# shz9/viprs

Hardware: AMD Instinct MI355X
Metric: SNP-updates/sec/E-step (1M SNPs, ~1700 LD blocks) (higher is better)
Workload: dtype f32

## Files before the change

viprs_amd/csrc/estep_panel.h:

```cpp
#pragma once
#include <type_traits>

#include "device_math.h"
#include "kernels_common.h"
#include "panel_loads.h"
#include "panel_models.h"

#ifndef PANEL_MIN_WAVES
#define PANEL_MIN_WAVES 2
#endif

namespace viprs {

#ifdef VIPRS_SWEEP_TRACE
__device__ unsigned long long g_sweep_trace[1 << 15][4];
__device__ unsigned int g_sweep_trace_n;
#endif

#ifdef VIPRS_PANEL_PROFILE
#define PPROF(slot, cond) do { if (TEAM && item == 0 && member < 2 && lane == 0 && p < 64 && (cond)) s_pprof[p][slot] = (unsigned)wall_clock64(); } while (0)
#else
#define PPROF(slot, cond) do { } while (0)
#endif

template <typename U> __host__ __device__ constexpr int panel_cols() { return sizeof(U) == 4 ? 4 : 8; }
template <typename U> __host__ __device__ constexpr int panel_team_cols() {
#ifdef PANEL_TEAM_CPL_F32
    return sizeof(U) == 4 ? PANEL_TEAM_CPL_F32 : 4;
#else
    return sizeof(U) == 4 ? 2 : 4;
#endif
}

constexpr int kFormSym = 1, kFormMirror = 2;

template <typename U, typename MODEL, int FORM, int NW, bool TEAM, int CPL>
__device__ __forceinline__ void panel_role(const EStepArgs<float>& A0, const int qcap, float* __restrict__ smem, const int wg) {
    constexpr bool MIR = FORM == kFormMirror;
    constexpr bool SUMS = FORM != kFormSym;
    const PanelLds lds(qcap, MODEL::kLaneParallel && !is_wide_mixture<MODEL>::value, MIR);
    float* lq = smem + lds.q();
    float* la = smem + lds.a();
    float* lT = smem + lds.diag_tiles();
    float* lTo = smem + lds.offdiag_tile();
    float* lmx = smem + lds.mix();
    float* led = smem + lds.ed();
    float* ls = smem + lds.s();
#ifdef PANEL_TEAM_STRIP_DEPTH
    constexpr int kDepth = TEAM ? PANEL_TEAM_STRIP_DEPTH : kStripRowsInFlight;
#else
    constexpr int kDepth = TEAM ? (kPanel / RawRow<U, CPL>::kWords < kPanel ? kPanel / RawRow<U, CPL>::kWords : kPanel) : kStripRowsInFlight;
#endif
    __shared__ int s_blk;
    __shared__ int s_tdone;
    __shared__ int s_ddone;

    const int tid = threadIdx.x;
    const int wave = __builtin_amdgcn_readfirstlane(tid >> 6);
    const int lane = tid & 63;
    const U* __restrict__ ldd = static_cast<const U*>(A0.ld_dense);
    ExpTab tab;
    tab.init();
    unsigned long long my_skipped = 0;
    const float dq = A0.dq;
    const int n_models = max(1, A0.n_active);

    constexpr int kSW = kPanel * CPL;
    const int TS = TEAM ? A0.team_size : 1;
    const int team = TEAM ? wg / TS : 0;
    const int member = TEAM ? wg % TS : 0;
    int team_iter = 0;

    for (;;) {
        int item;
        if (TEAM) {
            item = team + team_iter * A0.n_teams;
            ++team_iter;
        } else {
            if (tid == 0) {
                int it = atomicAdd(A0.counter, 1);
                if (A0.bottom_mod > 0 && it < A0.n_blocks * n_models) {
                    const bool bottom = (wg % A0.bottom_mod) == A0.bottom_mod - 1;
                    it = bottom ? A0.n_blocks * n_models - 1 - atomicAdd(A0.counter + 2, 1) : atomicAdd(A0.counter + 1, 1);
                }
                s_blk = it;
            }
            __syncthreads();
            item = s_blk;
            __syncthreads();
        }
        if (item >= A0.n_blocks * n_models) break;
        const int blk = item / n_models, model_slot = item - blk * n_models;
        if constexpr (IsGridColumn<MODEL>::value) {
            if (A0.group_cols) {
                const int on = A0.group_cols[(int64_t)A0.blk_group[blk] * A0.width + A0.active[model_slot]];
                if (__builtin_amdgcn_readfirstlane(on) == 0) continue;
            }
        }
        const EStepArgs<float> A = select_model(A0, model_slot);

        const BlockDesc bd = A.blocks[blk];
        const int64_t s0 = bd.start;
        const int b = bd.size;
#ifdef VIPRS_SWEEP_TRACE
        const unsigned long long trace_t0 = wall_clock64();
#endif
        unsigned long long* __restrict__ gran =
            TEAM ? A.granules + ((int64_t)model_slot * A.granule_rows + bd.gr_off) * kPanel : nullptr;
        const int stride = bd.stride;
        const U* __restrict__ base = ldd + bd.ld_off;
        const int np = (b + kPanel - 1) / kPanel;
        const int bpad = np * kPanel;
        const int nstrips_all = (bpad + kSW - 1) / kSW;
        const int n_own = TEAM ? (nstrips_all - member + TS - 1) / TS : nstrips_all;
        auto own = [&](int c) { return !TEAM || ((c / kSW) % TS) == member; };
        auto loc = [&](int c) { return TEAM ? ((c / kSW) / TS) * kSW + (c % kSW) : c; };
        auto glob = [&](int li) { return TEAM ? ((li / kSW) * TS + member) * kSW + (li % kSW) : li; };

        for (int li = tid; li < (TEAM ? n_own * kSW : bpad) + kStrip; li += NW * 64) {
            const int c = glob(li);
            const bool in = (!TEAM || li < n_own * kSW) && c < b;
            lq[li] = in ? A.q[s0 + c] : 0.0f;
            if (SUMS) ls[li] = 0.0f;
        }
        if (tid == 0) { s_tdone = 0; s_ddone = 0; }
        for (int i = tid; i < kPanel * kPanel / 4; i += NW * 64) {
            const int row = i >> 4, tcol = (i & 15) * 4;
            *reinterpret_cast<float4*>(lT + row * kPanel + tcol) = load4<U>(base + (int64_t)min(row, b - 1) * stride + tcol);
        }
        __syncthreads();

        float a_prev = 0.0f;

        typename MODEL::In nxt_in{};
        if (wave == 0) {
            const bool live0 = lane < b;
            nxt_in = MODEL::load(A, s0 + (live0 ? lane : 0), live0);
        }

#ifdef VIPRS_PANEL_PROFILE
        __shared__ unsigned s_pprof[64][8];
#endif
        if (wave == 0) {
#ifdef PANEL_CHAIN_PRIO
        __builtin_amdgcn_s_setprio(PANEL_CHAIN_PRIO);
#endif
        for (int p = 0; p < np + 1; ++p) {
            PPROF(0, true);
            {
                if (p < np) {
                    const int r0 = p * kPanel;
                    const int nrows = min(kPanel, b - r0);
                    const int64_t j = s0 + r0 + lane;
                    const bool live = lane < nrows;
                    const typename MODEL::In in = nxt_in;
                    {
                        const int rn = r0 + kPanel + lane;
                        const bool ln = rn < b;
                        nxt_in = MODEL::load(A, s0 + (ln ? rn : 0), ln);
                    }

                    float qc;
                    float q_own = 0.0f;
                    if (own(r0)) qc = lq[loc(r0 + lane)];
                    else qc = (r0 + lane < b) ? A.q[s0 + r0 + lane] : 0.0f;
                    if (TEAM && p >= 2 && (((p * kPanel) / kSW) % TS) != member) {
                        unsigned long long g = 0;
#ifdef PANEL_TIMING_NO_HANDOFF_WAIT
                        if (false)
#endif
                        for (unsigned spins = 0;; ++spins) {
                            g = __hip_atomic_load(gran + (int64_t)p * kPanel + lane, __ATOMIC_RELAXED,
                                                  __HIP_MEMORY_SCOPE_AGENT);
                            if (__all((unsigned)(g >> 32) == A.tag_base + (unsigned)(p + 1))) break;
                            if (spins > (1u << 22)) {
                                if (lane == 0) atomicExch(A.error, 1);
                                break;
                            }
                            if ((spins & 1023u) == 1023u &&
                                __hip_atomic_load(A.error, __ATOMIC_RELAXED, __HIP_MEMORY_SCOPE_AGENT) != 0) break;
                            __builtin_amdgcn_s_sleep(8);
                        }
                        qc = __uint_as_float((unsigned)g);
                    }
                    PPROF(1, true);
                    if (p > 0) {
                        {
                            float trow[kPanel];
#pragma unroll
                            for (int k = 0; k < kPanel; ++k) trow[k] = lTo[k * kPanel + lane];
                            if constexpr (sizeof(U) < 4 || MODEL::kLaneParallel) {
                                const float4* __restrict__ av4 = reinterpret_cast<const float4*>(la + ((p - 1) & 1) * kPanel);
                                float4 av[kPanel / 4];
#pragma unroll
                                for (int i = 0; i < kPanel / 4; ++i) av[i] = av4[i];
#pragma unroll
                                for (int k = 0; k < kPanel; ++k) {
                                    const float4 t = av[k >> 2];
                                    const float ak = (k & 3) == 0 ? t.x : (k & 3) == 1 ? t.y : (k & 3) == 2 ? t.z : t.w;
                                    qc = __builtin_fmaf(trow[k], ak, qc);
                                }
                            } else {
#pragma unroll
                                for (int k = 0; k < kPanel; ++k) qc = __builtin_fmaf(trow[k], rl(a_prev, k), qc);
                            }
                        }
                    }

                    {
                        if (lane == 0) *reinterpret_cast<volatile int*>(&s_tdone) = p + 1;
                    }
                    PPROF(2, true);
                    if constexpr (is_wide_mixture<MODEL>::value) {
                        constexpr int KMAX = MODEL::kMax;
                        const int K = in.K;
                        const int kc = min(lane, K - 1);
                        const bool comp = lane < K;
                        float dvec = 0.0f, avec = 0.0f;
                        const int64_t jlast = s0 + b - 1;
                        auto cptr = [&](const float* __restrict__ arr, int jj) {
                            return arr + min(s0 + r0 + jj, jlast) * K + kc;
                        };
                        static_assert(kChainPrefetch == 16 && kPanel == 64, "window indexing");
                        float rmm[kChainPrefetch], rsv[kChainPrefetch], rul[kChainPrefetch];
                        float rvec = in.beta - qc;
                        const float* __restrict__ DtW = lT + (p & 1) * kPanel * kPanel + lane;
#pragma unroll
                        for (int k = 0; k < kChainPrefetch; ++k) {
                            rmm[k] = *cptr(A.mu_mult, k);
                            rsv[k] = *cptr(A.shvt, k);
                            rul[k] = *cptr(A.u_logs, k);
                        }
#pragma unroll 1
                        for (int g = 0; g < kPanel / kChainPrefetch; ++g) {
#pragma unroll
                        for (int k = 0; k < kChainPrefetch; ++k) {
                            const int jj = kChainPrefetch * g + k;
                            const float drow_jj = DtW[jj * kPanel];
                            const float cmm = rmm[k], csv = rsv[k], cul = rul[k];
                            {
                                rmm[k] = *cptr(A.mu_mult, jj + kChainPrefetch);
                                rsv[k] = *cptr(A.shvt, jj + kChainPrefetch);
                                rul[k] = *cptr(A.u_logs, jj + kChainPrefetch);
                            }
                            const float lnp = rl(in.lnp, jj), eta_old = rl(in.eta_old, jj);
                            const float r = rl(rvec, jj);
                            const float mu = cmm * r;
                            const float t = csv * mu;
                            float u = __builtin_fmaf(t, t, cul);
                            u = (lane == K) ? lnp : u;
                            float mx = dpp_max_shr<1>(u);
                            mx = dpp_max_shr<2>(mx);
                            mx = dpp_max_shr<4>(mx);
                            mx = dpp_max_shr<8>(mx);
                            const float m_lo = rl(mx, 15), m_hi = rl(mx, K);
                            mx = (K >= 16) ? fmaxf(m_lo, m_hi) : m_hi;
                            float e = expf_glibc_nonpos<kLookupPerLane>(u - mx, tab);
                            e = (lane <= K) ? e : 0.0f;
                            static_assert((KMAX + 1) % 8 == 0, "chunks of 8 terms");
                            float ssum = 0.0f;
#pragma unroll
                            for (int c = 0; c < (KMAX + 1) / 8; ++c) {
                                int et[8];
#pragma unroll
                                for (int i = 0; i < 8; ++i) et[i] = __builtin_amdgcn_readlane(__float_as_int(e), 8 * c + i);
                                pin_sgprs(et);
#pragma unroll
                                for (int i = 0; i < 8; ++i) ssum = (c == 0 && i == 0) ? __int_as_float(et[0]) : ssum + __int_as_float(et[i]);
                            }
                            const float gam = comp ? e / ssum : 0.0f;
                            float d = -eta_old;
#pragma unroll
                            for (int c = 0; c < (KMAX + 1) / 8; ++c) {
                                int gt[8];
                                float mb[8];
#pragma unroll
                                for (int i = 0; i < 8; ++i) {
                                    gt[i] = __builtin_amdgcn_readlane(__float_as_int(gam), 8 * c + i);
                                    mb[i] = rl(mu, 8 * c + i);
                                }
                                pin_sgprs(gt);
#pragma unroll
                                for (int i = 0; i < 8; ++i) d = __builtin_fmaf(__int_as_float(gt[i]), mb[i], d);
                            }
                            const bool livej = jj < nrows;
                            const float a = livej ? dq * d : 0.0f;
                            if (comp && livej && member == 0) {
                                const int64_t o = (s0 + r0 + jj) * K + lane;
                                A.var_mu[o] = mu;
                                A.var_gamma[o] = gam;
                            }
                            int l = lane;
                            asm volatile("" : "+v"(l));
                            const bool me = (l == jj);
                            dvec = me ? d : dvec;
                            avec = me ? a : avec;
                            if (MIR) q_own = me ? qc : q_own;
                            qc = __builtin_fmaf(drow_jj, a, qc);
                            rvec = in.beta - qc;
                            if (!MIR) qc = (me && livej) ? qc - d : qc;
                        }
                        }
                        if (member == 0 && live) {
                            A.eta_diff[j] = dvec;
                            if (TEAM) stage_store(A.eta_out + j, in.eta_old + dvec); else A.eta[j] = in.eta_old + dvec;
                        }
                        a_prev = avec;
                        if (SUMS) led[(p & 1) * kPanel + lane] = live ? dvec : 0.0f;
                    } else if constexpr (MODEL::kLaneParallel) {
                        const int K = in.K;
                        float* __restrict__ Lmm = lmx;
                        float* __restrict__ Lsv = lmx + kPanel * kPanelMaxK;
                        float* __restrict__ Lul = lmx + 2 * kPanel * kPanelMaxK;
                        float* __restrict__ Lmu = lmx + 3 * kPanel * kPanelMaxK;
                        float* __restrict__ Lga = lmx + 4 * kPanel * kPanelMaxK;
#pragma unroll
                        for (int k = 0; k < kPanelMaxK; ++k) {
                            if (k < K) {
                                Lmm[lane * K + k] = in.mm[k];
                                Lsv[lane * K + k] = in.sv[k];
                                Lul[lane * K + k] = in.ulog[k];
                            }
                        }
                        __builtin_amdgcn_wave_barrier();
                        const int kc = min(lane, K - 1);
                        float cmm = Lmm[kc], csv = Lsv[kc], cul = Lul[kc];
                        float dvec = 0.0f, avec = 0.0f;
                        auto run_panel = [&](auto rounds_c, auto k4_c) {
                        constexpr int ROUNDS = decltype(rounds_c)::value;
                        constexpr bool K4 = decltype(k4_c)::value;
                        float rvec = in.beta - qc;
                        static_assert(kChainPrefetch == 16 && kPanel == 64, "group indexing");
                        const float* __restrict__ Dt = lT + (p & 1) * kPanel * kPanel + lane;
#pragma unroll 1
                        for (int g = 0; g < kPanel / kChainPrefetch; ++g) {
#pragma unroll
                        for (int k = 0; k < kChainPrefetch; ++k) {
                            const int jj = kChainPrefetch * g + k;
                            const float drow_jj = Dt[jj * kPanel];
                            const int jn = (jj + 1 < kPanel) ? jj + 1 : jj;
                            const float nmm = Lmm[jn * K + kc], nsv = Lsv[jn * K + kc], nul = Lul[jn * K + kc];
                            const float lnp = rl(in.lnp, jj), eta_old = rl(in.eta_old, jj);
                            const float r = rl(rvec, jj);
                            const float mu = cmm * r;
                            const float t = csv * mu;
                            float u = __builtin_fmaf(t, t, cul);
                            u = (lane == K) ? lnp : u;
                            float mub[ROUNDS];
#pragma unroll
                            for (int i = 0; i < ROUNDS; ++i) mub[i] = rl(mu, i);
                            float mx;
                            if constexpr (K4) {
                                int ut[5];
#pragma unroll
                                for (int i = 0; i < 5; ++i) ut[i] = __builtin_amdgcn_readlane(__float_as_int(u), i);
                                pin_sgprs(ut);
                                mx = __int_as_float(ut[0]);
#pragma unroll
                                for (int i = 1; i <= 4; ++i) mx = fmaxf(mx, __int_as_float(ut[i]));
                            } else {
                                mx = dpp_max_shr<1>(u);
                                mx = dpp_max_shr<2>(mx);
                                mx = dpp_max_shr<4>(mx);
                                mx = dpp_max_shr<8>(mx);
                                mx = rl(mx, K);
                            }
                            const float e = softmax_exp<MODEL::kExact, kLookupPerLane>(u - mx, tab);
                            const float e_t = (K4 || lane <= K) ? e : 0.0f;
                            int et[ROUNDS + 1];
#pragma unroll
                            for (int i = 0; i <= ROUNDS; ++i) et[i] = __builtin_amdgcn_readlane(__float_as_int(e_t), i);
                            pin_sgprs(et);
                            float ssum = __int_as_float(et[0]);
#pragma unroll
                            for (int i = 1; i <= ROUNDS; ++i) ssum += __int_as_float(et[i]);
                            const float gam = softmax_div<MODEL::kExact>(e, ssum);
                            const float gam_t = (K4 || lane < K) ? gam : 0.0f;
                            int gt[ROUNDS];
#pragma unroll
                            for (int i = 0; i < ROUNDS; ++i) gt[i] = __builtin_amdgcn_readlane(__float_as_int(gam_t), i);
                            pin_sgprs(gt);
                            float d = -eta_old;
#pragma unroll
                            for (int i = 0; i < ROUNDS; ++i) d = __builtin_fmaf(__int_as_float(gt[i]), mub[i], d);
                            const bool livej = jj < nrows;
                            const float a = livej ? dq * d : 0.0f;
                            if (lane < K) {
                                Lmu[jj * K + lane] = mu;
                                Lga[jj * K + lane] = gam;
                            }
                            int l = lane;
                            asm volatile("" : "+v"(l));
                            const bool me = (l == jj);
                            dvec = me ? d : dvec;
                            avec = me ? a : avec;
                            if (MIR) q_own = me ? qc : q_own;
                            qc = __builtin_fmaf(drow_jj, a, qc);
                            rvec = in.beta - qc;
                            if (!MIR) qc = (me && livej) ? qc - d : qc;
                            cmm = nmm; csv = nsv; cul = nul;
                        }
                        }
                        };
                        if (K == 4) run_panel(std::integral_constant<int, 4>{}, std::true_type{});
                        else if (K < 4) run_panel(std::integral_constant<int, 4>{}, std::false_type{});
                        else run_panel(std::integral_constant<int, kPanelMaxK>{}, std::false_type{});
                        __builtin_amdgcn_wave_barrier();
                        if (member == 0) {
                            const int64_t o = (s0 + r0) * K;
                            for (int i = lane; i < nrows * K; i += 64) {
                                A.var_mu[o + i] = Lmu[i];
                                A.var_gamma[o + i] = Lga[i];
                            }
                            if (live) {
                                A.eta_diff[j] = dvec;
                                if (TEAM) stage_store(A.eta_out + j, in.eta_old + dvec); else A.eta[j] = in.eta_old + dvec;
                            }
                        }
                        a_prev = avec;
                        if (SUMS) led[(p & 1) * kPanel + lane] = live ? dvec : 0.0f;
                    } else {
                        float qcap_v = 0.0f;
                        const float* __restrict__ Dt = lT + (p & 1) * kPanel * kPanel + lane;
                        unsigned long long lane_bit = 1ull;
                        float qf = qc;
    #pragma unroll
                        for (int jj = 0; jj < kPanel; ++jj) {
                            const float dr = Dt[jj * kPanel];
                            const float d = MODEL::template delta<kLookupLane>(in, qf, tab, jj);
                            const float dz = (MODEL::kHasSkip && fabsf(d) < Eps<float>::value) ? 0.0f : d;
                            const float az = dq * dz;
                            const float sa = rl(az, jj);
                            const float sdz = rl(dz, jj);
                            qcap_v = sel_mask(qcap_v, qc, lane_bit);
                            qf = __builtin_fmaf(dr, sa, qc);
                            qc = !MIR ? sel_mask(qf, qf - sdz, lane_bit) : qf;
                            asm volatile("s_lshl_b64 %0, %0, 1" : "+s"(lane_bit) : : "scc");
                        }
                        q_own = qcap_v;

                        PPROF(3, true);
                        bool skipped_lane;
                        float d_lane = 0.0f;
                        a_prev = MODEL::template finish<TEAM>(A, j, in, qcap_v, tab, live, member == 0, skipped_lane, &d_lane);
                        my_skipped += __popcll(__ballot(skipped_lane));
                        if (SUMS) led[(p & 1) * kPanel + lane] = d_lane;
                    }
                    la[(p & 1) * kPanel + lane] = a_prev;
                    if (own(r0)) lq[loc(r0 + lane)] = MIR ? q_own : qc;
                    PPROF(4, true);
                }
            }
            __syncthreads();
        }
        } else {
        for (int p = 0; p < np + 1; ++p) {
            {
                const int uw = wave - 1;
                auto stage_tiles = [&]() {
                if (p + 1 < np) {
                    float* __restrict__ T = lT + ((p + 1) & 1) * kPanel * kPanel;
                    const int trow = lane >> 4, tcol = (lane & 15) * 4;
                    const int row_base = (p + 1) * kPanel;
                    constexpr int kGroups = (kPanel / 4 + NW - 2) / (NW - 1);
                    float4 v[kGroups];
#pragma unroll
                    for (int g = 0; g < kGroups; ++g) {
                        const int row = 4 * min(uw + g * (NW - 1), kPanel / 4 - 1) + trow;
                        v[g] = load4<U>(base + (int64_t)min(row_base + row, b - 1) * stride + (p + 1) * kPanel + tcol);
                    }
                    float4 w[kGroups];
                    {
#pragma unroll
                        for (int g = 0; g < kGroups; ++g) {
                            const int row = 4 * min(uw + g * (NW - 1), kPanel / 4 - 1) + trow;
                            w[g] = load4<U>(base + (int64_t)min(p * kPanel + row, b - 1) * stride + (p + 1) * kPanel + tcol);
                        }
                    }
                    if (MIR && p > 0) {
                        while (*reinterpret_cast<volatile int*>(&s_ddone) < p) __builtin_amdgcn_s_sleep(1);
                    }
#pragma unroll
                    for (int g = 0; g < kGroups; ++g) {
                        const int i = uw + g * (NW - 1);
                        if (i < kPanel / 4) *reinterpret_cast<float4*>(T + (4 * i + trow) * kPanel + tcol) = v[g];
                    }
                    {
                        while (*reinterpret_cast<volatile int*>(&s_tdone) < p + 1) __builtin_amdgcn_s_sleep(1);
#pragma unroll
                        for (int g = 0; g < kGroups; ++g) {
                            const int i = uw + g * (NW - 1);
                            if (i < kPanel / 4) *reinterpret_cast<float4*>(lTo + (4 * i + trow) * kPanel + tcol) = w[g];
                        }
                    }
                }
                };
                const int pp = p - 1;
                const int rr0 = pp * kPanel;
                const int last_row = min(kPanel, b - rr0) - 1;
                const float avec = p > 0 ? la[(pp & 1) * kPanel + lane] : 0.0f;
                const int nstrips = (bpad + kSW - 1) / kSW;
                const bool any_a = __ballot(avec != 0.0f) != 0;
                const float edvec = (MIR && p > 0) ? led[(pp & 1) * kPanel + lane] : 0.0f;
                const bool any_ed = MIR && __ballot(edvec != 0.0f) != 0;
                const int s_pri = ((p + 1) * kPanel) / kSW;
                const int n_mine = (nstrips - member + TS - 1) / TS;
                auto do_strip = [&](int k) {
                    int st = member + k * TS, kl = k;
                    if (TEAM) {
                        const int k_pri = (s_pri % TS == member) ? (s_pri - member) / TS : 0;
                        kl = (k + k_pri) % n_mine;
                        st = member + kl * TS;
                    }
                    const int c = st * kSW + CPL * lane;
                    float* __restrict__ lq_c = lq + (TEAM ? kl * kSW + CPL * lane : c);
                    const int cp = c >> 6;
#if defined(PANEL_TIMING_NO_SECOND_PASS) && PANEL_TIMING_NO_SECOND_PASS + 0 >= 2
                    const bool active = (c < b) && cp > p;
#else
                    const bool active = (c < b) && cp != pp && cp != p;
#endif
                    auto hand_off = [&]() {
                        if (TEAM && st == s_pri && p + 1 < np && p + 1 >= 2) {
                            __builtin_amdgcn_wave_barrier();
                            const float v = lq[loc((p + 1) * kPanel + lane)];
                            const unsigned long long g =
                                ((unsigned long long)(A.tag_base + (unsigned)(p + 2)) << 32) | (unsigned long long)__float_as_uint(v);
                            __hip_atomic_store(gran + (int64_t)(p + 1) * kPanel + lane, g, __ATOMIC_RELAXED,
                                               __HIP_MEMORY_SCOPE_AGENT);
                        }
                    };
                    if constexpr (MIR) {
                        const bool left = cp < pp;
                        float* __restrict__ tgt = left ? ls + (TEAM ? kl * kSW + CPL * lane : c) : lq_c;
                        const bool any_l = __ballot(active && left) != 0, any_r = __ballot(active && !left) != 0;
                        if (any_l && any_r) {
                            const float fvec = left ? 1.0f : dq;
                            if (any_ed && active) {
                                if (last_row == kPanel - 1)
                                    strip_update<U, CPL, true, kDepth, true>(base + (int64_t)rr0 * stride + c, stride, last_row, edvec, tgt, fvec);
                                else
                                    strip_update<U, CPL, false, kDepth, true>(base + (int64_t)rr0 * stride + c, stride, last_row, edvec, tgt, fvec);
                            }
                        } else {
                            float mvec = any_l ? edvec : avec;
                            asm volatile("" : "+v"(mvec));
                            if ((any_l ? any_ed : any_a) && active) {
                                if (last_row == kPanel - 1)
                                    strip_update<U, CPL, true, kDepth>(base + (int64_t)rr0 * stride + c, stride, last_row, mvec, tgt);
                                else
                                    strip_update<U, CPL, false, kDepth>(base + (int64_t)rr0 * stride + c, stride, last_row, mvec, tgt);
                            }
                        }
                        if (k == uw) PPROF(6, wave == 1);
                        hand_off();
                    } else {
                        if (any_a && active) {
                            if (last_row == kPanel - 1)
                                strip_update<U, CPL, true, kDepth>(base + (int64_t)rr0 * stride + c, stride, last_row, avec, lq_c);
                            else
                                strip_update<U, CPL, false, kDepth>(base + (int64_t)rr0 * stride + c, stride, last_row, avec, lq_c);
                        }
                        if (k == uw) PPROF(6, wave == 1);
                        hand_off();
                    }
                };
                if (MIR && p > 0 && uw == NW - 2) {
#ifdef PANEL_TIMING_NO_SECOND_PASS
                    if (false) {
#else
                    if (any_ed && own(rr0)) {
#endif
                        float* __restrict__ sp = ls + loc(rr0 + lane);
                        *sp = diag_lower_update(lT + (pp & 1) * kPanel * kPanel, edvec, *sp, lane);
                    }
                    if (lane == 0) *reinterpret_cast<volatile int*>(&s_ddone) = p;
                }
                stage_tiles();
                PPROF(5, wave == 1);
                if (p > 0) {
                    for (int k = uw; k < n_mine; k += NW - 1) do_strip(k);
                }
            }
            PPROF(7, wave == 1);
            __syncthreads();
        }
        }
#ifdef VIPRS_PANEL_PROFILE
        if (TEAM && item == 0 && member < 2 && tid == 0) {
            for (int p = 0; p < np && p < 64; p += (p < 4 || p > np - 4) ? 1 : 8) {
                const unsigned t = s_pprof[p][0];
                printf("m%d phase %2d @%7u: granule %4d T-apply %4d loop %5d replay %5d end %5d | upd: staged %5d pri %5d all %5d (x10ns)\n",
                       member, p, t - s_pprof[0][0], (int)(s_pprof[p][1] - t), (int)(s_pprof[p][2] - t), (int)(s_pprof[p][3] - t),
                       (int)(s_pprof[p][4] - t), (int)(s_pprof[p][4] - t), (int)(s_pprof[p][5] - t), (int)(s_pprof[p][6] - t),
                       (int)(s_pprof[p][7] - t));
            }
        }
#endif
        {
            for (int li = tid; li < (TEAM ? n_own * kSW : b); li += NW * 64) {
                const int i = glob(li);
                if (i < b) {
                    const float v = SUMS ? lq[li] + A.dq * ls[li] : lq[li];
                    if (TEAM) stage_store(A.q_out + s0 + i, v); else A.q[s0 + i] = v;
                }
            }
        }
        if (TEAM) {
            asm volatile("s_waitcnt vmcnt(0)" ::: "memory");
            __syncthreads();
            if (tid == 0) s_blk = (atomicAdd(A.arrive + item, 1) == TS - 1) ? 1 : 0;
            __syncthreads();
            const bool last = s_blk != 0;
            if (last) {
                for (int i = tid; i < b; i += NW * 64) {
                    A.eta[s0 + i] = __hip_atomic_load(A.eta_out + s0 + i, __ATOMIC_RELAXED, __HIP_MEMORY_SCOPE_AGENT);
                    A.q[s0 + i] = __hip_atomic_load(A.q_out + s0 + i, __ATOMIC_RELAXED, __HIP_MEMORY_SCOPE_AGENT);
                }
                if (tid == 0) atomicExch(A.arrive + item, 0);
            }
        }
        __syncthreads();
#ifdef VIPRS_SWEEP_TRACE
        if (tid == 0) {
            const unsigned k = atomicAdd(&g_sweep_trace_n, 1u);
            if (k < (1u << 15)) {
                g_sweep_trace[k][0] = ((unsigned long long)blockIdx.x << 32) | (unsigned)(TEAM ? 1 : 0);
                g_sweep_trace[k][1] = (unsigned long long)b;
                g_sweep_trace[k][2] = trace_t0;
                g_sweep_trace[k][3] = wall_clock64();
            }
        }
#endif
    }
    if (lane == 0 && my_skipped && member == 0) atomicAdd(A0.skipped, my_skipped);
}

struct SweepArgs {
    EStepArgs<float> cls[3];
    int32_t qcap[3];
    int32_t n_wg[2];
    int32_t narrow0;
    int32_t* done;
    unsigned long long* skipped_last;
};

template <typename U, typename MODEL, int FORM, int NW, int CPL>
__global__ __launch_bounds__(NW * 64, PANEL_MIN_WAVES) void estep_sweep_kernel(SweepArgs S) {
    extern __shared__ __attribute__((aligned(16))) float smem[];
    const int wg = blockIdx.x;
    const int team_cls = wg < S.n_wg[0] ? 0 : (wg < S.n_wg[0] + S.n_wg[1] ? 1 : 2);
    if (team_cls < 2) {
        constexpr bool kNarrowForm = FORM == kFormMirror && sizeof(U) < 4;
        constexpr int CPL_N = (MODEL::kLaneParallel || !kNarrowForm) ? CPL : panel_team_cols<U>();
        const int wg_t = wg - (team_cls ? S.n_wg[0] : 0);
        if (CPL_N != CPL && team_cls == 0 && S.narrow0)
            panel_role<U, MODEL, FORM, NW, true, CPL_N>(S.cls[0], S.qcap[0], smem, wg_t);
        else
            panel_role<U, MODEL, FORM, NW, true, CPL>(S.cls[team_cls], S.qcap[team_cls], smem, wg_t);
        __syncthreads();
    }
    if (S.cls[2].n_blocks > 0) panel_role<U, MODEL, FORM, NW, false, CPL>(S.cls[2], S.qcap[2], smem, wg);
    __syncthreads();
    if (threadIdx.x == 0) {
        if (atomicAdd(S.done, 1) == (int)gridDim.x - 1) {
            S.cls[2].counter[0] = 0; S.cls[2].counter[1] = 0; S.cls[2].counter[2] = 0;
            atomicExch(S.skipped_last, atomicExch(S.cls[2].skipped, 0ull));
            atomicExch(S.done, 0);
        }
    }
}

}
```

viprs_amd/csrc/kernels_common.h:

```cpp
#pragma once
#include <hip/hip_runtime.h>
#include <stdint.h>

#if (defined(PANEL_TIMING_NO_HANDOFF_WAIT) || \
    defined(PANEL_TIMING_NO_SECOND_PASS) || \
    defined(PANEL_NW) || \
    defined(PANEL_STRIP_DEPTH) || \
    defined(PANEL_MIN_WAVES) || \
    defined(PANEL_TEAM_STRIP_DEPTH) || \
    defined(PANEL_TEAM_CPL_F32) || \
    defined(PANEL_CHAIN_PRIO) || \
    defined(VIPRS_GRID_MFMA_CHAIN) || \
    defined(VIPRS_GRID_PROFILE) || \
    defined(VIPRS_TILE_PROFILE) || \
    defined(VIPRS_SWEEP_TRACE) || \
    defined(VIPRS_PANEL_PROFILE)) && \
    !defined(VIPRS_EXPERIMENTAL)
#error "experiment switch defined without -DVIPRS_EXPERIMENTAL (see kernels_common.h)"
#endif
#ifdef VIPRS_EXPERIMENTAL
#define VIPRS_BF_VIPRS_EXPERIMENTAL " VIPRS_EXPERIMENTAL"
#else
#define VIPRS_BF_VIPRS_EXPERIMENTAL ""
#endif
#ifdef PANEL_TIMING_NO_HANDOFF_WAIT
#define VIPRS_BF_PANEL_TIMING_NO_HANDOFF_WAIT " PANEL_TIMING_NO_HANDOFF_WAIT"
#else
#define VIPRS_BF_PANEL_TIMING_NO_HANDOFF_WAIT ""
#endif
#ifdef PANEL_TIMING_NO_SECOND_PASS
#define VIPRS_BF_PANEL_TIMING_NO_SECOND_PASS " PANEL_TIMING_NO_SECOND_PASS"
#else
#define VIPRS_BF_PANEL_TIMING_NO_SECOND_PASS ""
#endif
#ifdef PANEL_NW
#define VIPRS_BF_PANEL_NW " PANEL_NW"
#else
#define VIPRS_BF_PANEL_NW ""
#endif
#ifdef PANEL_STRIP_DEPTH
#define VIPRS_BF_PANEL_STRIP_DEPTH " PANEL_STRIP_DEPTH"
#else
#define VIPRS_BF_PANEL_STRIP_DEPTH ""
#endif
#ifdef PANEL_MIN_WAVES
#define VIPRS_BF_PANEL_MIN_WAVES " PANEL_MIN_WAVES"
#else
#define VIPRS_BF_PANEL_MIN_WAVES ""
#endif
#ifdef PANEL_TEAM_STRIP_DEPTH
#define VIPRS_BF_PANEL_TEAM_STRIP_DEPTH " PANEL_TEAM_STRIP_DEPTH"
#else
#define VIPRS_BF_PANEL_TEAM_STRIP_DEPTH ""
#endif
#ifdef PANEL_TEAM_CPL_F32
#define VIPRS_BF_PANEL_TEAM_CPL_F32 " PANEL_TEAM_CPL_F32"
#else
#define VIPRS_BF_PANEL_TEAM_CPL_F32 ""
#endif
#ifdef PANEL_CHAIN_PRIO
#define VIPRS_BF_PANEL_CHAIN_PRIO " PANEL_CHAIN_PRIO"
#else
#define VIPRS_BF_PANEL_CHAIN_PRIO ""
#endif
#ifdef VIPRS_GRID_MFMA_CHAIN
#define VIPRS_BF_VIPRS_GRID_MFMA_CHAIN " VIPRS_GRID_MFMA_CHAIN"
#else
#define VIPRS_BF_VIPRS_GRID_MFMA_CHAIN ""
#endif
#ifdef VIPRS_GRID_PROFILE
#define VIPRS_BF_VIPRS_GRID_PROFILE " VIPRS_GRID_PROFILE"
#else
#define VIPRS_BF_VIPRS_GRID_PROFILE ""
#endif
#ifdef VIPRS_TILE_PROFILE
#define VIPRS_BF_VIPRS_TILE_PROFILE " VIPRS_TILE_PROFILE"
#else
#define VIPRS_BF_VIPRS_TILE_PROFILE ""
#endif
#ifdef VIPRS_SWEEP_TRACE
#define VIPRS_BF_VIPRS_SWEEP_TRACE " VIPRS_SWEEP_TRACE"
#else
#define VIPRS_BF_VIPRS_SWEEP_TRACE ""
#endif
#ifdef VIPRS_PANEL_PROFILE
#define VIPRS_BF_VIPRS_PANEL_PROFILE " VIPRS_PANEL_PROFILE"
#else
#define VIPRS_BF_VIPRS_PANEL_PROFILE ""
#endif
#define VIPRS_TU_BUILD_FLAGS VIPRS_BF_VIPRS_EXPERIMENTAL VIPRS_BF_PANEL_TIMING_NO_HANDOFF_WAIT VIPRS_BF_PANEL_TIMING_NO_SECOND_PASS VIPRS_BF_PANEL_NW VIPRS_BF_PANEL_STRIP_DEPTH VIPRS_BF_PANEL_MIN_WAVES VIPRS_BF_PANEL_TEAM_STRIP_DEPTH VIPRS_BF_PANEL_TEAM_CPL_F32 VIPRS_BF_PANEL_CHAIN_PRIO VIPRS_BF_VIPRS_GRID_MFMA_CHAIN VIPRS_BF_VIPRS_GRID_PROFILE VIPRS_BF_VIPRS_TILE_PROFILE VIPRS_BF_VIPRS_SWEEP_TRACE VIPRS_BF_VIPRS_PANEL_PROFILE

namespace viprs {
void register_build_flags(const char* flags);
struct BuildFlagsRegistrar { explicit BuildFlagsRegistrar(const char* f) { register_build_flags(f); } };
}

namespace viprs {

constexpr int kPanel = 64;
constexpr int kStrip = 256;

constexpr int kPanelMaxK = 8;
constexpr int kPanelWideMaxK = 31;
constexpr int kMixLdsFloats = 5 * kPanel * kPanelMaxK;
struct PanelLds {
    int qcap;
    bool mix_scratch, mirror;
    __host__ __device__ constexpr PanelLds(int qcap_, bool mix_scratch_, bool mirror_)
        : qcap(qcap_), mix_scratch(mix_scratch_), mirror(mirror_) {}
    __host__ __device__ constexpr int q() const { return 0; }
    __host__ __device__ constexpr int a() const { return qcap; }
    __host__ __device__ constexpr int diag_tiles() const { return a() + 2 * kPanel; }
    __host__ __device__ constexpr int offdiag_tile() const { return diag_tiles() + 2 * kPanel * kPanel; }
    __host__ __device__ constexpr int mix() const { return offdiag_tile() + kPanel * kPanel; }
    __host__ __device__ constexpr int ed() const { return mix() + (mix_scratch ? kMixLdsFloats : 0); }
    __host__ __device__ constexpr int s() const { return ed() + 2 * kPanel; }
    __host__ __device__ constexpr int total_floats() const { return mirror ? s() + qcap : ed(); }
};
constexpr int kMaxMixtureK = 64;
constexpr int kGridModels = 32;
constexpr int kGridResOwners = 6, kGridResSlots = 2;
constexpr int kGridResMaxCols = kGridResOwners * kGridResSlots * 2 * kPanel;
constexpr int kBandMaxRingPanels = 256;

struct BlockDesc {
    int32_t start;
    int32_t size;
    int32_t stride;
    int32_t kind;
    int64_t ld_off;
    int64_t gr_off;
    int32_t band_left;
    int32_t band_right;
};

template <typename T>
struct EStepArgs {
    const BlockDesc* blocks;
    int32_t n_blocks;
    int32_t* counter;
    int32_t bottom_mod;
    unsigned long long* granules;
    uint32_t tag_base;
    int32_t* arrive;
    int32_t* error;
    int32_t n_teams;
    int32_t team_size;
    int64_t granule_rows;
    unsigned long long* skipped;
    const int32_t* lb;
    const int64_t* rowstart;
    const int32_t* rowlen;
    const void* ld_rows;
    const void* ld_dense;
    int64_t ld_zero_off;
    const T* std_beta;
    const T* u_logs;
    const T* shvt;
    const T* mu_mult;
    const T* log_null_pi;
    T* var_gamma;
    T* var_mu;
    T* eta;
    T* q;
    T* eta_diff;
    T* eta_out;
    T* q_out;
    T dq;
    int32_t low_memory;
    int32_t width;
    int64_t m;
    const int32_t* active;
    int32_t n_active;
    const int32_t* blk_group;
    const uint8_t* group_cols;
    const int32_t* group_lists;
};
constexpr int kGroupListStride = 1 + kGridModels;

template <typename T>
__device__ __forceinline__ EStepArgs<T> select_model(const EStepArgs<T>& A0, int model_slot) {
    EStepArgs<T> A = A0;
    if (A0.n_active > 0) {
        const int64_t off = (int64_t)A0.active[model_slot] * A0.m;
        A.var_gamma += off; A.var_mu += off; A.eta += off; A.q += off; A.eta_diff += off;
        A.u_logs += off; A.shvt += off; A.mu_mult += off;
        if (A.eta_out) { A.eta_out += off; A.q_out += off; }
    }
    return A;
}

}
```

viprs_amd/csrc/launch_panel.inc:

```
#include "internal.h"
#include "estep_panel.h"

static viprs::BuildFlagsRegistrar viprs_tu_build_flags_(VIPRS_TU_BUILD_FLAGS);

namespace viprs {

template <typename U, int NW>
int launch_panel_nw(viprs_plan* P, EStepArgs<float> A, int model) {
    constexpr int CPL = panel_cols<U>();
    const bool exact = P->math_mode == VIPRS_MATH_EXACT;
    const bool upper = P->low_memory != 0;
    const bool mirror = upper;
    if (upper) { const int rc = ensure_upper_storage(P, true); if (rc != VIPRS_OK) return rc; }
    const int n_models = std::max(1, A.n_active);
    const int* team_of = ((model == kPanelMixture || model == kPanelMixtureWide) && !sched_config().team_env) ? sched_config().class_team_mix
                                                                             : sched_config().class_team;
    const void* kfn = nullptr;
#define PK(MODEL) (upper ? (const void*)estep_sweep_kernel<U, MODEL, kFormMirror, NW, CPL>       \
                          : (const void*)estep_sweep_kernel<U, MODEL, kFormSym, NW, CPL>)
    if (model == kPanelGridColumn) kfn = exact ? PK(GridColumnModel<true>) : PK(GridColumnModel<false>);
    else if (model == kPanelMixture) kfn = exact ? PK(MixtureModel<true>) : PK(MixtureModel<false>);
    else if (model == kPanelMixtureWide) kfn = A.width <= 15 ? PK(MixtureWideModel<15>) : PK(MixtureWideModel<31>);
    else kfn = exact ? PK(SpikeSlabModel<true>) : PK(SpikeSlabModel<false>);
#undef PK
    P->math_used |= (exact || model == kPanelMixtureWide) ? 1 : 2;

    const int n_team_blocks = P->class_begin[2];
    const int64_t ng = P->n_granule_rows * kPanel * (int64_t)n_models;
    if (P->d_granules.n < (size_t)ng) {
        HIP_TRY(hipStreamSynchronize(P->stream));
        HIP_TRY(P->d_granules.alloc((size_t)ng));
        HIP_TRY(hipMemsetAsync(P->d_granules.p, 0, sizeof(unsigned long long) * (size_t)ng, P->stream));
    }
    const size_t n_arrive = (size_t)n_team_blocks * (size_t)n_models + 1;
    if (P->d_arrive.n < n_arrive) {
        HIP_TRY(hipStreamSynchronize(P->stream));
        HIP_TRY(P->d_arrive.alloc(n_arrive));
        HIP_TRY(hipMemsetAsync(P->d_arrive.p, 0, sizeof(int32_t) * n_arrive, P->stream));
    }
    P->granule_gen = (P->granule_gen + 1) & 0xFFFFFu;
    if (P->granule_gen == 0) {
        if (P->d_granules.n) HIP_TRY(hipMemsetAsync(P->d_granules.p, 0, sizeof(unsigned long long) * P->d_granules.n, P->stream));
        P->granule_gen = 1;
    }
    A.granules = P->d_granules.p;
    A.tag_base = P->granule_gen << 12;

    SweepArgs S{};
    S.done = P->d_arrive.p + (n_arrive - 1);
    S.skipped_last = P->d_skipped.p + 1;
    size_t shmem = 0;
    for (int c = 0; c < 3; ++c) {
        EStepArgs<float>& C = S.cls[c];
        C = A;
        const int begin = P->class_begin[c], end = P->class_begin[c + 1];
        C.blocks = P->d_dense.p + begin;
        C.n_blocks = end - begin;
        if (A.blk_group) C.blk_group = A.blk_group + begin;
        C.counter = c < 2 ? P->d_counters.p + 4 + c : P->d_counters.p + 16;
        C.arrive = P->d_arrive.p + (c == 1 ? (size_t)(P->class_begin[1] - P->class_begin[0]) * (size_t)n_models : 0);
        C.bottom_mod = 0;
        C.team_size = c < 2 ? team_of[c] : 1;
        if (c == 0 && P->team0 > 0 && team_of == sched_config().class_team) C.team_size = P->team0;
        if (c == 0 && team_of == sched_config().class_team_mix) {
            const int64_t room = (int64_t)P->n_cu * 2 * 5 / 8;
            while (C.team_size > 4 && (int64_t)(end - begin) * n_models * C.team_size > room) C.team_size -= 4;
        }
        C.n_teams = 0;
        S.qcap[c] = 0;
        if (end > begin) {
            const int max_b = P->dense_h[begin].size;
            auto lds_bytes = [&](int qcap) {
                return (size_t)PanelLds(qcap, model == kPanelMixture, mirror).total_floats() * sizeof(float);
            };
            for (;;) {
                S.qcap[c] = (max_b + kPanel - 1) / kPanel * kPanel + kStrip;
                if (c < 2) {
                    const bool narrow = upper && sizeof(U) < 4 && c == 0 && C.team_size >= 8 && model != kPanelMixture && model != kPanelMixtureWide;
                    if (c == 0) S.narrow0 = narrow ? 1 : 0;
                    const int kSW = kPanel * (narrow ? panel_team_cols<U>() : CPL);
                    const int n_strips = ((max_b + kPanel - 1) / kPanel * kPanel + kSW - 1) / kSW;
                    S.qcap[c] = (n_strips + C.team_size - 1) / C.team_size * kSW + kStrip;
                }
                if (c < 2 && lds_bytes(S.qcap[c]) > 160 * 1024 && C.team_size < 16) { ++C.team_size; continue; }
                break;
            }
            shmem = std::max(shmem, lds_bytes(S.qcap[c]));
        }
    }
    if (shmem == 0) return P->timing.launcher_start();
    if (shmem > 160 * 1024) return fail(VIPRS_EUNSUPPORTED, "LD block too large for the LDS-resident panel kernel");
    if (shmem > 48 * 1024)
        HIP_TRY(hipFuncSetAttribute(kfn, hipFuncAttributeMaxDynamicSharedMemorySize, (int)shmem));
    int per_cu = 0;
    HIP_TRY(hipOccupancyMaxActiveBlocksPerMultiprocessor(&per_cu, kfn, NW * 64, shmem));
    per_cu = std::max(1, per_cu);
    if (const char* f = getenv("VIPRS_MAX_WG_PER_CU")) per_cu = std::max(1, std::min(per_cu, atoi(f)));
    const int capacity = P->n_cu * per_cu;

    const int64_t n_small = (int64_t)S.cls[2].n_blocks * n_models;
    const int team_budget = n_small > 0 ? capacity * 5 / 8 : capacity;
    int team_wgs = 0;
    {
        const double es = (double)sizeof(U);
        auto class_time = [&](int c, int n_teams) {
            const EStepArgs<float>& C = S.cls[c];
            const int64_t n_items = (int64_t)C.n_blocks * n_models;
            double t = 0.0;
            for (int64_t i = 0; i < n_items; i += n_teams) {
                const double sz = (double)P->dense_h[(size_t)(P->class_begin[c] + i / n_models)].size;
                t += std::max(sz * 135e-9, sz * sz * es / (C.team_size * 16e9));
            }
            return t;
        };
        const int64_t items[2] = {(int64_t)S.cls[0].n_blocks * n_models, (int64_t)S.cls[1].n_blocks * n_models};
        const int TS0 = S.cls[0].team_size, TS1 = S.cls[1].team_size;
        int best[2] = {0, 0};
        const int64_t key[6] = {items[0], items[1], TS0, TS1, team_budget, (int64_t)sizeof(U)};
        if (std::equal(key, key + 6, P->team_split.key)) {
            best[0] = P->team_split.best[0];
            best[1] = P->team_split.best[1];
        } else if (items[0] > 0 && items[1] > 0) {
            double best_t = 1e30;
            const int max0 = (int)std::min<int64_t>(items[0], std::max(1, (team_budget - TS1) / TS0));
            for (int n0 = 1; n0 <= max0; ++n0) {
                const int n1 = (int)std::min<int64_t>(items[1], std::max(1, (team_budget - n0 * TS0) / TS1));
                const double t = std::max(class_time(0, n0), class_time(1, n1));
                if (t < best_t * (1.0 - 1e-9)) { best_t = t; best[0] = n0; best[1] = n1; }
            }
        } else if (items[0] > 0) {
            best[0] = (int)std::min<int64_t>(items[0], std::max(1, team_budget / TS0));
        } else if (items[1] > 0) {
            best[1] = (int)std::min<int64_t>(items[1], std::max(1, team_budget / TS1));
        }
        std::copy(key, key + 6, P->team_split.key);
        P->team_split.best[0] = best[0];
        P->team_split.best[1] = best[1];
        for (int c = 0; c < 2; ++c) {
            EStepArgs<float>& C = S.cls[c];
            C.n_teams = best[c];
            S.n_wg[c] = C.n_teams * C.team_size;
            team_wgs += S.n_wg[c];
        }
    }
    if (team_wgs > capacity) return fail(VIPRS_EUNSUPPORTED, "team size exceeds the resident workgroups of the device");
    int grid = (int)std::min<int64_t>(capacity, (int64_t)team_wgs + n_small);
    grid = std::max(grid, team_wgs);
    if (n_small >= 4 * (int64_t)P->n_cu) S.cls[2].bottom_mod = sched_config().bottom_mod;

    void* params[] = {(void*)&S};
    if (team_wgs > 0) { const int rc = team_launch_gate(P); if (rc != VIPRS_OK) return rc; }
    { const int rc = P->timing.launcher_start(); if (rc != VIPRS_OK) return rc; }
    HIP_TRY(hipLaunchKernel(kfn, dim3(grid), dim3(NW * 64), params, shmem, P->stream));
    if (team_wgs > 0) { const int rc = team_launch_done(P); if (rc != VIPRS_OK) return rc; }
    return VIPRS_OK;
}

template <typename U>
int launch_panel(viprs_plan* P, EStepArgs<float> A, int model) {
#ifdef PANEL_NW
    return launch_panel_nw<U, PANEL_NW>(P, A, model);
#else
    return launch_panel_nw<U, kClassWaves[0]>(P, A, model);
#endif
}

template int launch_panel<PANEL_U>(viprs_plan*, EStepArgs<float>, int);

#if defined(VIPRS_SWEEP_TRACE)
#define PANEL_TRACE_FN2(tag) viprs_debug_sweep_trace_##tag
#define PANEL_TRACE_FN(tag) PANEL_TRACE_FN2(tag)
extern "C" int PANEL_TRACE_FN(PANEL_TAG)(unsigned long long* out, int capacity) {
    unsigned n = 0;
    if (hipDeviceSynchronize() != hipSuccess) return -1;
    if (hipMemcpyFromSymbol(&n, HIP_SYMBOL(g_sweep_trace_n), sizeof(n)) != hipSuccess) return -1;
    n = std::min<unsigned>(n, std::min<unsigned>(1u << 15, (unsigned)capacity));
    if (n && hipMemcpyFromSymbol(out, HIP_SYMBOL(g_sweep_trace), (size_t)n * 32) != hipSuccess) return -1;
    const unsigned zero = 0;
    (void)hipMemcpyToSymbol(HIP_SYMBOL(g_sweep_trace_n), &zero, sizeof(zero));
    return (int)n;
}
#endif

}
```

viprs_amd/csrc/panel_loads.h:

```cpp
#pragma once
#include "kernels_common.h"

namespace viprs {

template <typename U> __device__ __forceinline__ float4 load4(const U* p);
template <> __device__ __forceinline__ float4 load4<float>(const float* p) {
    return *reinterpret_cast<const float4*>(p);
}
template <> __device__ __forceinline__ float4 load4<int8_t>(const int8_t* p) {
    const int w = *reinterpret_cast<const int*>(p);
    return make_float4((float)(int8_t)(w), (float)(int8_t)(w >> 8), (float)(int8_t)(w >> 16),
                       (float)(int8_t)(w >> 24));
}
template <> __device__ __forceinline__ float4 load4<int16_t>(const int16_t* p) {
    const int2 w = *reinterpret_cast<const int2*>(p);
    return make_float4((float)(int16_t)(w.x), (float)(int16_t)(w.x >> 16), (float)(int16_t)(w.y),
                       (float)(int16_t)(w.y >> 16));
}

template <int N> __device__ __forceinline__ void pin_sgprs(int (&v)[N]) {
    static_assert(N == 4 || N == 5 || N == 8 || N == 9, "chain lengths of the K <= 8 mixture step");
    if constexpr (N == 4) asm volatile("" : "+s"(v[0]), "+s"(v[1]), "+s"(v[2]), "+s"(v[3]));
    if constexpr (N == 5) asm volatile("" : "+s"(v[0]), "+s"(v[1]), "+s"(v[2]), "+s"(v[3]), "+s"(v[4]));
    if constexpr (N == 8) asm volatile("" : "+s"(v[0]), "+s"(v[1]), "+s"(v[2]), "+s"(v[3]), "+s"(v[4]), "+s"(v[5]), "+s"(v[6]), "+s"(v[7]));
    if constexpr (N == 9) asm volatile("" : "+s"(v[0]), "+s"(v[1]), "+s"(v[2]), "+s"(v[3]), "+s"(v[4]), "+s"(v[5]), "+s"(v[6]), "+s"(v[7]),
                                       "+s"(v[8]));
}
template <int N> __device__ __forceinline__ float dpp_max_shr(float x) {
    float r;
    if (N == 1) asm("s_nop 1\n\tv_max_f32_dpp %0, %1, %1 row_shr:1 row_mask:0xf bank_mask:0xf" : "=v"(r) : "v"(x), "0"(x));
    if (N == 2) asm("s_nop 1\n\tv_max_f32_dpp %0, %1, %1 row_shr:2 row_mask:0xf bank_mask:0xf" : "=v"(r) : "v"(x), "0"(x));
    if (N == 4) asm("s_nop 1\n\tv_max_f32_dpp %0, %1, %1 row_shr:4 row_mask:0xf bank_mask:0xf" : "=v"(r) : "v"(x), "0"(x));
    if (N == 8) asm("s_nop 1\n\tv_max_f32_dpp %0, %1, %1 row_shr:8 row_mask:0xf bank_mask:0xf" : "=v"(r) : "v"(x), "0"(x));
    return r;
}

__device__ __forceinline__ float sel_mask(float a, float b, unsigned long long m) {
    float r;
    asm("v_cndmask_b32_e64 %0, %1, %2, %3" : "=v"(r) : "v"(a), "v"(b), "s"(m));
    return r;
}

__device__ __forceinline__ void stage_store(float* p, float v) {
    __hip_atomic_store(p, v, __ATOMIC_RELAXED, __HIP_MEMORY_SCOPE_AGENT);
}

__device__ __forceinline__ float rl(float v, int lane) {
    return __int_as_float(__builtin_amdgcn_readlane(__float_as_int(v), lane));
}

template <typename U, int CPL> struct RawRow {
    static constexpr int kWords = CPL * (int)sizeof(U) / 4;
    static_assert(CPL * sizeof(U) % 4 == 0 && (kWords == 1 || kWords == 2 || kWords == 4), "1, 2 or 4 dwords per lane and row");
    unsigned w[kWords];
    __device__ __forceinline__ float get(int i) const {
        if constexpr (sizeof(U) == 4) return __uint_as_float(w[i]);
        else if constexpr (sizeof(U) == 1) return static_cast<float>(static_cast<int8_t>(w[i >> 2] >> (8 * (i & 3))));
        else return static_cast<float>(static_cast<int16_t>(w[i >> 1] >> (16 * (i & 1))));
    }
};
template <typename U, int CPL> __device__ __forceinline__ RawRow<U, CPL> load_raw(const U* p) {
    RawRow<U, CPL> r;
    if constexpr (RawRow<U, CPL>::kWords == 1) {
        r.w[0] = *reinterpret_cast<const unsigned*>(p);
    } else if constexpr (RawRow<U, CPL>::kWords == 2) {
        const uint2 t = *reinterpret_cast<const uint2*>(p);
        r.w[0] = t.x; r.w[1] = t.y;
    } else {
        const uint4 t = *reinterpret_cast<const uint4*>(p);
        r.w[0] = t.x; r.w[1] = t.y; r.w[2] = t.z; r.w[3] = t.w;
    }
    return r;
}

constexpr int kChainPrefetch = 16;
#ifndef PANEL_STRIP_DEPTH
#define PANEL_STRIP_DEPTH 16
#endif
constexpr int kStripRowsInFlight = PANEL_STRIP_DEPTH;


template <typename U, int CPL, bool FULL, int DEPTH = kStripRowsInFlight, bool MIXED = false>
__device__ __forceinline__ void strip_update(const U* __restrict__ rowp, int stride, int last_row, float avec,
                                             float* __restrict__ lq_c, float fvec = 1.0f) {
    static_assert(kPanel % DEPTH == 0, "panel must be a whole number of prefetch groups");
    float qv[CPL];
#pragma unroll
    for (int i = 0; i < CPL; ++i) qv[i] = lq_c[i];
    RawRow<U, CPL> buf[DEPTH];
#pragma unroll
    for (int k = 0; k < DEPTH; ++k)
        buf[k] = load_raw<U, CPL>(rowp + (int64_t)(FULL ? k : min(k, last_row)) * stride);
#pragma unroll 1
    for (int g = 0; g < kPanel / DEPTH - 1; ++g) {
#pragma unroll
        for (int k = 0; k < DEPTH; ++k) {
            const RawRow<U, CPL> v = buf[k];
            const int rn = DEPTH * (g + 1) + k;
            buf[k] = load_raw<U, CPL>(rowp + (int64_t)(FULL ? rn : min(rn, last_row)) * stride);
            const float a = MIXED ? fvec * rl(avec, DEPTH * g + k) : rl(avec, DEPTH * g + k);
#pragma unroll
            for (int i = 0; i < CPL; ++i) qv[i] = __builtin_fmaf(v.get(i), a, qv[i]);
            __builtin_amdgcn_sched_barrier(0);
        }
    }
#pragma unroll
    for (int k = 0; k < DEPTH; ++k) {
        const RawRow<U, CPL> v = buf[k];
        const float a = MIXED ? fvec * rl(avec, kPanel - DEPTH + k) : rl(avec, kPanel - DEPTH + k);
#pragma unroll
        for (int i = 0; i < CPL; ++i) qv[i] = __builtin_fmaf(v.get(i), a, qv[i]);
    }
#pragma unroll
    for (int i = 0; i < CPL; ++i) lq_c[i] = qv[i];
}

__device__ __forceinline__ float diag_lower_update(const float* __restrict__ tile, float edvec, float sv, int lane) {
#pragma unroll 16
    for (int jr = 0; jr < kPanel; ++jr) {
        const float t = __builtin_fmaf(tile[jr * kPanel + lane], rl(edvec, jr), sv);
        sv = lane < jr ? t : sv;
    }
    return sv;
}

}
```

Baseline: 1.454 billion.

## Stage off-diagonal panel tile in padded double-buffered LDS for non-team mirror blocks

For non-team, mirror-form, f32 spike-slab/grid models, the off-diagonal tile is now written into a padded (stride kPanel+1), double-buffered LDS layout. This lets the chain wave read its column without bank conflicts and stage the next tile without waiting on s_tdone. A dedicated sub-wave applies the previous tile's mirrored row update, tracked by a new s_sdone flag, and that strip is skipped in the regular strip pass. The path costs extra LDS (qcap is reduced by one panel) and is enabled only when occupancy does not drop, with a VIPRS_SUB_LDS env override.

```diff
diff --git a/viprs_amd/csrc/estep_panel.h b/viprs_amd/csrc/estep_panel.h
--- a/viprs_amd/csrc/estep_panel.h
+++ b/viprs_amd/csrc/estep_panel.h
@@ -35,10 +35,14 @@
 constexpr int kFormSym = 1, kFormMirror = 2;
 
 template <typename U, typename MODEL, int FORM, int NW, bool TEAM, int CPL>
-__device__ __forceinline__ void panel_role(const EStepArgs<float>& A0, const int qcap, float* __restrict__ smem, const int wg) {
+__device__ __forceinline__ void panel_role(const EStepArgs<float>& A0, const int qcap, float* __restrict__ smem, const int wg,
+                                           const bool sub_lds) {
     constexpr bool MIR = FORM == kFormMirror;
     constexpr bool SUMS = FORM != kFormSym;
     const PanelLds lds(qcap, MODEL::kLaneParallel && !is_wide_mixture<MODEL>::value, MIR);
+    constexpr bool kSubLds = !TEAM && MIR && sizeof(U) == 4 && !MODEL::kLaneParallel && !is_wide_mixture<MODEL>::value;
+    constexpr int kSubWave = NW >= 4 ? NW - 3 : NW - 2;
+    const bool sub = kSubLds && sub_lds;
     float* lq = smem + lds.q();
     float* la = smem + lds.a();
     float* lT = smem + lds.diag_tiles();
@@ -54,6 +58,7 @@
     __shared__ int s_blk;
     __shared__ int s_tdone;
     __shared__ int s_ddone;
+    __shared__ int s_sdone;
 
     const int tid = threadIdx.x;
     const int wave = __builtin_amdgcn_readfirstlane(tid >> 6);
@@ -117,13 +122,15 @@
         auto loc = [&](int c) { return TEAM ? ((c / kSW) / TS) * kSW + (c % kSW) : c; };
         auto glob = [&](int li) { return TEAM ? ((li / kSW) * TS + member) * kSW + (li % kSW) : li; };
 
-        for (int li = tid; li < (TEAM ? n_own * kSW : bpad) + kStrip; li += NW * 64) {
+        const int n_init = (TEAM ? n_own * kSW : bpad) + kStrip;
+        for (int li = tid; li < (kSubLds ? min(n_init, qcap) : n_init); li += NW * 64) {
             const int c = glob(li);
             const bool in = (!TEAM || li < n_own * kSW) && c < b;
             lq[li] = in ? A.q[s0 + c] : 0.0f;
             if (SUMS) ls[li] = 0.0f;
         }
         if (tid == 0) { s_tdone = 0; s_ddone = 0; }
+        if constexpr (kSubLds) { if (tid == 0) s_sdone = 0; }
         for (int i = tid; i < kPanel * kPanel / 4; i += NW * 64) {
             const int row = i >> 4, tcol = (i & 15) * 4;
             *reinterpret_cast<float4*>(lT + row * kPanel + tcol) = load4<U>(base + (int64_t)min(row, b - 1) * stride + tcol);
@@ -184,7 +191,22 @@
                         qc = __uint_as_float((unsigned)g);
                     }
                     PPROF(1, true);
-                    if (p > 0) {
+                    bool applied = false;
+                    if constexpr (kSubLds) {
+                        if (p > 0 && sub) {
+                            applied = true;
+                            const int bsel = (p - 1) & 1;
+                            const float* __restrict__ t0 = smem + PanelSubLds::row(lds, bsel, 0) + lane;
+                            const float* __restrict__ t63 = smem + PanelSubLds::row(lds, bsel, kPanel - 1) + lane;
+                            float trow[kPanel];
+#pragma unroll
+                            for (int k = 0; k < kPanel - 1; ++k) trow[k] = t0[k * kSubStride];
+                            trow[kPanel - 1] = t63[0];
+#pragma unroll
+                            for (int k = 0; k < kPanel; ++k) qc = __builtin_fmaf(trow[k], rl(a_prev, k), qc);
+                        }
+                    }
+                    if (p > 0 && !applied) {
                         {
                             float trow[kPanel];
 #pragma unroll
@@ -485,7 +507,22 @@
                         const int i = uw + g * (NW - 1);
                         if (i < kPanel / 4) *reinterpret_cast<float4*>(T + (4 * i + trow) * kPanel + tcol) = v[g];
                     }
-                    {
+                    bool staged = false;
+                    if constexpr (kSubLds) {
+                        if (sub) {
+                            staged = true;
+                            if (p >= 2) while (*reinterpret_cast<volatile int*>(&s_sdone) < p) __builtin_amdgcn_s_sleep(1);
+#pragma unroll
+                            for (int g = 0; g < kGroups; ++g) {
+                                const int i = uw + g * (NW - 1);
+                                if (i < kPanel / 4) {
+                                    float* __restrict__ r = smem + PanelSubLds::row(lds, p & 1, 4 * i + trow) + tcol;
+                                    r[0] = w[g].x; r[1] = w[g].y; r[2] = w[g].z; r[3] = w[g].w;
+                                }
+                            }
+                        }
+                    }
+                    if (!staged) {
                         while (*reinterpret_cast<volatile int*>(&s_tdone) < p + 1) __builtin_amdgcn_s_sleep(1);
 #pragma unroll
                         for (int g = 0; g < kGroups; ++g) {
@@ -518,7 +555,8 @@
 #if defined(PANEL_TIMING_NO_SECOND_PASS) && PANEL_TIMING_NO_SECOND_PASS + 0 >= 2
                     const bool active = (c < b) && cp > p;
 #else
-                    const bool active = (c < b) && cp != pp && cp != p;
+                    bool active = (c < b) && cp != pp && cp != p;
+                    if constexpr (kSubLds) active = active && !(sub && cp == pp - 1);
 #endif
                     auto hand_off = [&]() {
                         if (TEAM && st == s_pri && p + 1 < np && p + 1 >= 2) {
@@ -575,6 +613,15 @@
                         *sp = diag_lower_update(lT + (pp & 1) * kPanel * kPanel, edvec, *sp, lane);
                     }
                     if (lane == 0) *reinterpret_cast<volatile int*>(&s_ddone) = p;
+                }
+                if constexpr (kSubLds) {
+                    if (sub && p > 0 && uw == kSubWave) {
+                        if (p >= 2 && any_ed) {
+                            float* __restrict__ sp = ls + rr0 - kPanel + lane;
+                            *sp = offdiag_row_update(smem + PanelSubLds::row(lds, p & 1, lane), edvec, *sp);
+                        }
+                        if (lane == 0) *reinterpret_cast<volatile int*>(&s_sdone) = p;
+                    }
                 }
                 stage_tiles();
                 PPROF(5, wave == 1);
@@ -640,6 +687,7 @@
     EStepArgs<float> cls[3];
     int32_t qcap[3];
     int32_t n_wg[2];
+    int32_t sub_lds;
     int32_t narrow0;
     int32_t* done;
     unsigned long long* skipped_last;
@@ -655,12 +703,12 @@
         constexpr int CPL_N = (MODEL::kLaneParallel || !kNarrowForm) ? CPL : panel_team_cols<U>();
         const int wg_t = wg - (team_cls ? S.n_wg[0] : 0);
         if (CPL_N != CPL && team_cls == 0 && S.narrow0)
-            panel_role<U, MODEL, FORM, NW, true, CPL_N>(S.cls[0], S.qcap[0], smem, wg_t);
+            panel_role<U, MODEL, FORM, NW, true, CPL_N>(S.cls[0], S.qcap[0], smem, wg_t, S.sub_lds != 0);
         else
-            panel_role<U, MODEL, FORM, NW, true, CPL>(S.cls[team_cls], S.qcap[team_cls], smem, wg_t);
+            panel_role<U, MODEL, FORM, NW, true, CPL>(S.cls[team_cls], S.qcap[team_cls], smem, wg_t, S.sub_lds != 0);
         __syncthreads();
     }
-    if (S.cls[2].n_blocks > 0) panel_role<U, MODEL, FORM, NW, false, CPL>(S.cls[2], S.qcap[2], smem, wg);
+    if (S.cls[2].n_blocks > 0) panel_role<U, MODEL, FORM, NW, false, CPL>(S.cls[2], S.qcap[2], smem, wg, S.sub_lds != 0);
     __syncthreads();
     if (threadIdx.x == 0) {
         if (atomicAdd(S.done, 1) == (int)gridDim.x - 1) {
diff --git a/viprs_amd/csrc/kernels_common.h b/viprs_amd/csrc/kernels_common.h
--- a/viprs_amd/csrc/kernels_common.h
+++ b/viprs_amd/csrc/kernels_common.h
@@ -117,6 +117,17 @@
     __host__ __device__ constexpr int s() const { return ed() + 2 * kPanel; }
     __host__ __device__ constexpr int total_floats() const { return mirror ? s() + qcap : ed(); }
 };
+constexpr int kSubStride = kPanel + 1;
+constexpr int kSubBufFloats = (kPanel - 1) * kSubStride + kPanel;
+struct PanelSubLds {
+    __host__ __device__ static constexpr int extra_floats() { return (kSubBufFloats + kPanel + 3) / 4 * 4; }
+    __host__ __device__ static constexpr int row(const PanelLds& L, int buf, int row) {
+        return buf ? L.total_floats() + row * kSubStride
+                   : (row < kPanel - 1 ? L.offdiag_tile() + row * kSubStride : L.total_floats() + kSubBufFloats);
+    }
+};
+static_assert((kPanel - 1) * kSubStride <= kPanel * kPanel, "rows 0 .. 62 of buffer 0 fit the plain tile's place");
+
 constexpr int kMaxMixtureK = 64;
 constexpr int kGridModels = 32;
 constexpr int kGridResOwners = 6, kGridResSlots = 2;
diff --git a/viprs_amd/csrc/launch_panel.inc b/viprs_amd/csrc/launch_panel.inc
--- a/viprs_amd/csrc/launch_panel.inc
+++ b/viprs_amd/csrc/launch_panel.inc
@@ -50,6 +50,9 @@
     S.done = P->d_arrive.p + (n_arrive - 1);
     S.skipped_last = P->d_skipped.p + 1;
     size_t shmem = 0;
+    auto lds_bytes = [&](int qcap) {
+        return (size_t)PanelLds(qcap, model == kPanelMixture, mirror).total_floats() * sizeof(float);
+    };
     for (int c = 0; c < 3; ++c) {
         EStepArgs<float>& C = S.cls[c];
         C = A;
@@ -70,9 +73,6 @@
         S.qcap[c] = 0;
         if (end > begin) {
             const int max_b = P->dense_h[begin].size;
-            auto lds_bytes = [&](int qcap) {
-                return (size_t)PanelLds(qcap, model == kPanelMixture, mirror).total_floats() * sizeof(float);
-            };
             for (;;) {
                 S.qcap[c] = (max_b + kPanel - 1) / kPanel * kPanel + kStrip;
                 if (c < 2) {
@@ -90,6 +90,24 @@
     }
     if (shmem == 0) return P->timing.launcher_start();
     if (shmem > 160 * 1024) return fail(VIPRS_EUNSUPPORTED, "LD block too large for the LDS-resident panel kernel");
+    if (mirror && sizeof(U) == 4 && (model == kPanelSpikeSlab || model == kPanelGridColumn) && S.qcap[2] > 0) {
+        const size_t shmem_sub =
+            std::max(shmem, lds_bytes(S.qcap[2] - kPanel) + PanelSubLds::extra_floats() * sizeof(float));
+        bool on = shmem_sub <= 160 * 1024;
+        if (const char* f = getenv("VIPRS_SUB_LDS")) on = on && atoi(f) != 0;
+        if (on) {
+            int per_cu_plain = 0, per_cu_sub = 0;
+            HIP_TRY(hipFuncSetAttribute(kfn, hipFuncAttributeMaxDynamicSharedMemorySize, (int)std::max<size_t>(shmem_sub, 48 * 1024)));
+            HIP_TRY(hipOccupancyMaxActiveBlocksPerMultiprocessor(&per_cu_plain, kfn, NW * 64, shmem));
+            HIP_TRY(hipOccupancyMaxActiveBlocksPerMultiprocessor(&per_cu_sub, kfn, NW * 64, shmem_sub));
+            on = per_cu_sub >= std::min(per_cu_plain, PANEL_MIN_WAVES);
+        }
+        if (on) {
+            S.sub_lds = 1;
+            shmem = shmem_sub;
+            S.qcap[2] -= kPanel;
+        }
+    }
     if (shmem > 48 * 1024)
         HIP_TRY(hipFuncSetAttribute(kfn, hipFuncAttributeMaxDynamicSharedMemorySize, (int)shmem));
     int per_cu = 0;
diff --git a/viprs_amd/csrc/panel_loads.h b/viprs_amd/csrc/panel_loads.h
--- a/viprs_amd/csrc/panel_loads.h
+++ b/viprs_amd/csrc/panel_loads.h
@@ -124,4 +124,10 @@
     return sv;
 }
 
+__device__ __forceinline__ float offdiag_row_update(const float* __restrict__ rowp, float edvec, float sv) {
+#pragma unroll 16
+    for (int j = 0; j < kPanel; ++j) sv = __builtin_fmaf(rowp[j], rl(edvec, j), sv);
+    return sv;
 }
+
+}
```

Measured after the change: 1.507 billion (median of 6 runs). +3.7%, better.
